# felixlutz/carla-social-force-model

Hardware: AMD Instinct MI355X
Metric: sfm_ticks_per_s (higher is better)
Workload: dtype f32

## Files before the change

carla-social-force-model_amd/csrc/sfm_capi.hip:

```cpp
#include "sfm_capi_common.h"

using namespace sfm;

constexpr int GEO_SLICES_MAX = 16;


struct DevGeo {
    DevBuf<int> off;
    DevBuf<float2> pts;
    DevBuf<float4> ctr;
    DevBuf<float4> seg;
    int K = 0;
    int P = 0;
    PinnedBuf<char> stage;
    std::vector<int> off_host;
    bool lazy = false;
    bool lazy_off = false;
};

struct FsmDev {
    bool on = false;
    int n = 0;
    DevBuf<uint8_t> mode;
    DevBuf<float> target, initial, crossing, margin, next;
// ... 830 lines not shown
    return sa;
}

constexpr int PHASE_FULL = 0, PHASE_BEGIN = 1, PHASE_END = 2;
constexpr int LIST_ALL = 0, LIST_OWN = 1, LIST_REMOTE = 2;

static int fused_launch(SfmHandle* h, uint32_t flags, int mode, int* sl) {
    const int n_g = (h->n_t + 1) / 2;
    const size_t rows = (size_t)n_g * (size_t)h->N_pad;
    TickArgs a;
    fill_args(h, a, flags);
    const bool geo = a.geo != nullptr;
    int slices = 0, nw = 16;
    const int n_pair = fused_pair_workgroups(n_g);
    if (geo) {
        slices = h->n_t <= 64 ? 4 : 2;
        if (h->n_t >= 6) slices = std::max(slices, std::min(FUSED_GEO_SLICES_MAX, (256 - n_pair) / h->n_t));
        if (n_pair + h->n_t * slices > 512) nw = 8;
    }
    const size_t grow = (size_t)FUSED_GEO_SLICES_MAX * (size_t)h->N_pad;
    if (geo && a.adv.M > 0) {
        float4* c_in = mode ? h->fused.dyn_ctr_alt : h->dynamics.ctr;
        float2* p_in = mode ? h->fused.dyn_pts_alt : h->dynamics.pts;
        a.dynamics.ctr = c_in; a.dynamics.pts = p_in;
        a.adv.ctr = c_in; a.adv.pts = p_in;
        a.adv.ctr_out = mode ? h->dynamics.ctr : h->fused.dyn_ctr_alt;
        a.adv.pts_out = mode ? h->dynamics.pts : h->fused.dyn_pts_alt;
    }
    const FusedArgs f{h->fused.fslab + (size_t)(*sl ^ 1) * rows, h->fused.fslab + (size_t)*sl * rows,
                      h->z3 ? h->fused.fslabz + (size_t)(*sl ^ 1) * rows : nullptr, h->z3 ? h->fused.fslabz + (size_t)*sl * rows : nullptr,
                      h->own, h->fused.own_alt, n_g, h->n_t, n_g % 8 == 0 ? 1 : 0,
                      geo ? h->fused.fgeo + (size_t)(*sl ^ 1) * grow : nullptr, geo ? h->fused.fgeo + (size_t)*sl * grow : nullptr, slices,
                      geo ? h->n_t * slices : 0, n_pair, mode};
    HIP_TRY(h, launch_fused_tick(h->rad, a, f, h->stream, nw));
    if (mode != 0) {
        h->cur ^= 1;
        swap(h->own, h->fused.own_alt);
        if (geo && a.adv.M > 0) {
            swap(h->dynamics.ctr, h->fused.dyn_ctr_alt);
            swap(h->dynamics.pts, h->fused.dyn_pts_alt);
        }
    }
    *sl ^= 1;
    return SFM_OK;
}

static int fused_reserve(SfmHandle* h) {
    const size_t need = (size_t)2 * (size_t)((h->n_t + 1) / 2) * (size_t)h->N_pad;
    FusedDev& f = h->fused;
    if (need > f.fslab.cap()) HIP_TRY(h, f.fslab.alloc(need));
    if (h->z3 && need > f.fslabz.cap()) HIP_TRY(h, f.fslabz.alloc(need));
    if (f.own_alt.cap() < (size_t)h->cap) HIP_TRY(h, f.own_alt.alloc((size_t)h->cap));
    const size_t gneed = (size_t)2 * FUSED_GEO_SLICES_MAX * (size_t)h->N_pad;
    if (gneed > f.fgeo.cap()) HIP_TRY(h, f.fgeo.alloc(gneed));
    if (h->dyn_boxes && h->dynamics.K > 0) {
        if (f.dyn_ctr_alt.cap() != h->dynamics.ctr.cap()) HIP_TRY(h, f.dyn_ctr_alt.alloc(h->dynamics.ctr.cap()));
        if (f.dyn_pts_alt.cap() != h->dynamics.pts.cap()) HIP_TRY(h, f.dyn_pts_alt.alloc(h->dynamics.pts.cap()));
    }
    return SFM_OK;
}

static int run_fused(SfmHandle* h, int ticks, uint32_t flags, bool carry, bool geo) {
    int rc = fused_reserve(h);
    if (rc) return rc;
    snprintf(h->variant, sizeof(h->variant), geo ? "sfm_fused_tick_kernel(geo)" : "sfm_fused_tick_kernel");
    if (h->timing_on) HIP_TRY(h, hipEventRecord(h->ev0, h->stream));
    int sl = carry ? h->carry_sl : 0;
// ... 712 lines not shown
```

carla-social-force-model_amd/csrc/sfm_capi_common.h:

```cpp
#pragma once
#include "sfm_devbuf.h"
#include "sfm_device.h"
#include "sfm_hip.h"

#include <algorithm>
#include <cmath>
#include <numeric>
#include <cstdio>
#include <cstdlib>
#include <cstring>
#include <limits>
#include <string>
#include <vector>

namespace sfm {
hipError_t launch_tick(int ipw, int team, bool z3, bool rad, const TickArgs& a, hipStream_t st);
hipError_t launch_arrived(const float4* pk, const float4* own, int N, float thr2, uint8_t* mask, hipStream_t st);
hipError_t launch_sym_list(const TickArgs& a, const SymArgs& sa, hipStream_t st, int partners = 0, bool count_is_zero = false);
hipError_t launch_sym_pair(bool rad, const TickArgs& a, const SymArgs& sa, hipStream_t st);
hipError_t launch_sym_epilogue(bool rad, const TickArgs& a, const SymArgs& sa, hipStream_t st);
hipError_t launch_fused_tick(bool rad, const TickArgs& a, const FusedArgs& f, hipStream_t st, int waves);
int fused_pair_workgroups(int n_g);
hipError_t launch_sym_pair_geo(bool rad, const TickArgs& a, const SymArgs& sa, hipStream_t st);
int sym_item_count(int n_t);
hipError_t launch_strip_bounds(const float4* box, const float* vmax, int n_t, int tps, int n_strips, float4* sbox, float* svmax,
                               hipStream_t st);
hipError_t launch_tile_strip_bounds(const float4* pk, int N, int n_t, int tps, int n_strips, float4* box, float* vmax, float4* sbox,
                                    float* svmax, hipStream_t st);
hipError_t launch_geometry(bool rad, const TickArgs& a, hipStream_t st);
hipError_t launch_modes(const TickArgs& a, hipStream_t st);
struct ReorderBufs { unsigned long long *key64_in, *key64_out; uint32_t *row_a, *row_b, *key32_in, *key32_out; void* temp; size_t temp_bytes; };
size_t reorder_temp_bytes(int N);
hipError_t launch_resort(const float4* pk, int N, int strip_rows, const ReorderBufs& b, hipStream_t st);
hipError_t launch_resort_blocks(const float4* pk, int N, const BlockPlan& pl, const ReorderBufs& b, hipStream_t st);
hipError_t launch_unpack_geo(const char* block, float4* ctr, int K, float2* pts, int P, int* off, bool with_off, hipStream_t st);
hipError_t launch_unpack_rows(const char* block, size_t b_own, size_t b_zv, size_t b_rr, size_t b_cm, int n_pad, float4* pk0,
                              float4* pk1, float4* own, float2* zv0, float2* zv1, float* radius, uint8_t* crossing, uint32_t* draws,
                              const char* geo_block, float4* ctr, int K, float2* pts, int P, int* off, bool with_off, hipStream_t st);
hipError_t launch_gather(const uint32_t* src, int N, const float4* pk_in, float4* pk_out, const float2* zv_in, float2* zv_out,
                         const float4* own_in, float4* own_out, const float* rad_in, float* rad_out, const uint8_t* cr_in,
                         uint8_t* cr_out, const uint32_t* dr_in, uint32_t* dr_out, const uint32_t* id_in, uint32_t* id_out,
                         hipStream_t st);
hipError_t launch_tile_bounds(const float4* pk, const float2* zv, int N, float4* box, float* vmax, hipStream_t st, int t_lo = 0,
                              int t_hi = -1);
int probe_dpp_direction(hipStream_t st);
hipError_t launch_batch_tick(bool z3, bool ext, bool modes, bool spawn, bool steer, const BatchArgs& a, int B, hipStream_t st);
hipError_t launch_batch_park_unborn(const int* scene_off, const uint8_t* born, float4* pk, float2* zv, int B, hipStream_t st);
hipError_t launch_batch_place_tracks(const BatchTracks& t, const int* off, const float2* local, float4* ctr, float2* pts, int M,
                                     hipStream_t st);
hipError_t launch_batch_restart(const BatchRestart& r, int scenes, hipStream_t st);
hipError_t launch_batch_observe(const ObserveArgs& a, int B, hipStream_t st);
hipError_t launch_dynamic_boxes(float4* ctr, const int* off, const float2* local, const float2* rot, float2* pts, int M,
                                float dt, int advance, hipStream_t st);

// ... 38 lines not shown
```

carla-social-force-model_amd/csrc/sfm_device.h:

```cpp
#pragma once
#include <hip/hip_runtime.h>
#include <stdint.h>

namespace sfm {

constexpr int WAVE = 64;
constexpr int BLOCK = 256;
constexpr int WAVES_PER_BLOCK = BLOCK / WAVE;
constexpr int TILE_J = BLOCK;
constexpr float TINY = 1e-30f;
constexpr float COINCIDENT_RINV = 1e14f;

constexpr float FAR_AWAY = 3.0e15f;
constexpr float FAR_STEP = 1.0e12f;
constexpr float BOX_LIMIT = 1.0e14f;
constexpr float NEAR_LIMIT = 1.0e12f;

struct IxConst {
    float lam;
    float eg;
    float c1;
    float k1;
    float k2;
    float negA;
// ... 105 lines not shown
    int t_lo, t_hi;
    int zero_count;
    uint32_t* idx;
    uint32_t row_base;
    uint32_t cap_pairs;
    struct SpillArgs* spill;
    int tick_serial;
};

struct SpillArgs {
    long long* ovf;
    int n_pad;
    int tick;
};

constexpr int FUSED_GEO_SLICES_MAX = 8;
struct alignas(16) FusedArgs {
    const float2* slab_prev;
    float2* slab_next;
    const float* slabz_prev;
    float* slabz_next;
    const float4* own_cur;
    float4* own_next;
    int n_g;
    int n_t;
    int blocked;
    const float2* geo_prev;
    float2* geo_next;
    int geo_slices;
    int n_geo_wg;
    int n_pair_wg;
    int mode;
};

constexpr int BATCH_MAX_N = 1024;
struct BatchParams {
    IxConst ped, stat, dyn;
    float border_a, border_nlb;
    float inv_tau, dt, max_speed_factor;
    int en_acc, en_ped, en_border, en_static, en_dynamic;
    int rad;
    int pad;
};
struct BatchGeo {
    const int* item_off;
    const int* off;
    const float2* pts;
    const float4* ctr;
};
struct BatchStream {
    uint32_t seed;
    float world_side;
    float arrive_thr2;
    float pad;
};
struct BatchModeScene {
    float arrive_thr2;
    float veh_ext_x, veh_ext_y;
    int despawn_on_arrival;
};
struct BatchModes {
    uint8_t* mode;
    float* target;
    const float4* speeds;
    const int* wp_off;
    const float2* wp_xy;
// ... 90 lines not shown
```

carla-social-force-model_amd/csrc/sfm_kernels.hip:

```cpp
#include "sfm_device.h"
#include "sfm_interaction.h"

#include <algorithm>
#include <type_traits>

namespace sfm {

typedef float v2f __attribute__((ext_vector_type(2)));
__device__ __forceinline__ v2f bcast(float v) { v2f r; r.x = v; r.y = v; return r; }
template <bool RAD, bool CUT>
__device__ __forceinline__ bool moussaid_planar_pk(const IxConst& c, v2f pj, v2f uj, v2f Ti, v2f Ui, float rsum, float reach2, v2f& term) {
    const v2f dd = pj - Ti;
    const float d2 = fmaf(dd.x, dd.x, dd.y * dd.y);
    if (CUT && !__any(!(d2 > reach2))) return false;
    v2f sq, rr;
    sq.x = d2;
    rr.x = rsq(d2);
    const v2f Dv = __builtin_elementwise_fma(dd, __builtin_shufflevector(rr, rr, 0, 0), Ui - uj);
    const float D2 = fmaf(Dv.x, Dv.x, fmaf(Dv.y, Dv.y, TINY));
    sq.y = D2;
    rr.y = rsq(D2);
    const float rD = rr.y;
    float aL = 0.f;
    if (CUT) {
// ... 1517 lines not shown
        rc[(3 * 3 + 0) * n + i] = fsx; rc[(3 * 3 + 1) * n + i] = fsy; rc[(3 * 3 + 2) * n + i] = 0.f;
        rc[(4 * 3 + 0) * n + i] = fdx; rc[(4 * 3 + 1) * n + i] = fdy; rc[(4 * 3 + 2) * n + i] = 0.f;
        rc[(5 * 3 + 0) * n + i] = Fx;  rc[(5 * 3 + 1) * n + i] = Fy;  rc[(5 * 3 + 2) * n + i] = Fz;
    }
}

constexpr int GROUP = 2 * WAVE;

template <bool RAD, int NW, bool Z3>
struct FusedShared {
    float4 st[2 * GROUP];
    float rad[2 * GROUP];
    float2 q[Z3 ? 1 : NW / 2][2 * GROUP];
    float2 part[2 * GROUP];
    int badrow[2 * GROUP];
    int any;
    float2 fi[NW][WAVE];
    float2 fj[NW][WAVE];
    float fiz[Z3 ? NW : 1][WAVE];
    float fjz[Z3 ? NW : 1][WAVE];
    float2 fi2[NW][WAVE];
    float fi2z[Z3 ? NW : 1][WAVE];
    float4 trav[4][2 * WAVE];
    float radt[RAD ? 4 : 1][2 * WAVE];
    float2 stz[Z3 ? 2 * GROUP : 1];
    float2 travz[Z3 ? 4 : 1][2 * WAVE];
    float partz[Z3 ? 2 * GROUP : 1];
    __device__ __forceinline__ float2 (*qv())[2 * GROUP] { return Z3 ? reinterpret_cast<float2 (*)[2 * GROUP]>(&fi[0][0]) : q; }
    __device__ __forceinline__ float (*qzv())[2 * GROUP] {
        return reinterpret_cast<float (*)[2 * GROUP]>(reinterpret_cast<char*>(&fi[0][0]) + sizeof(float2) * (NW / 2) * 2 * GROUP);
    }
};

template <bool RAD, int NW, bool Z3, bool GEO>
__global__ __launch_bounds__(NW * WAVE, (NW == 8 && Z3) ? 6 : 8) void sfm_fused_tick_kernel(const TickArgs a, const FusedArgs f) {
    constexpr int PARTS = NW / 2;
    constexpr int SPW = 4 * WAVE / NW;
    constexpr int D = NW / 8;
    using Sh = FusedShared<RAD, NW, Z3>;
    constexpr size_t LDS = (GEO && sizeof(GeoShared<NW>) > sizeof(Sh)) ? sizeof(GeoShared<NW>) : sizeof(Sh);
    __shared__ __attribute__((aligned(16))) char smem[LDS];
    Sh& sh = *reinterpret_cast<Sh*>(smem);
    static_assert(!Z3 || (offsetof(Sh, fjz) + sizeof(sh.fjz) - offsetof(Sh, fi) == (sizeof(float2) + sizeof(float)) * (NW / 2) * 2 * GROUP &&
                          offsetof(Sh, fj) == offsetof(Sh, fi) + sizeof(sh.fi) && offsetof(Sh, fiz) == offsetof(Sh, fj) + sizeof(sh.fj) &&
                          offsetof(Sh, fjz) == offsetof(Sh, fiz) + sizeof(sh.fiz)),
                  "3-D: q / qz are laid over fi | fj | fiz | fjz, which must be one block of exactly that size");
    const int tid = threadIdx.x;
    const int lane = tid & (WAVE - 1);
    const int wave = uniform(tid >> 6);
    const int n_g = f.n_g, n_t = f.n_t;
    const int half_up = (n_g + 1) >> 1;
    const bool geo_role = GEO && (int)blockIdx.x < f.n_geo_wg;
    const int bid = (int)blockIdx.x - (GEO ? f.n_geo_wg : 0);
    if (GEO && bid >= f.n_pair_wg) {
        const int k = (bid - f.n_pair_wg) * NW + wave;
        if (k < a.adv.M) advance_vehicle(a.adv, k, lane, true);
        return;
    }
    const int geo_tile = geo_role ? (int)blockIdx.x % n_t : 0, geo_slice = geo_role ? (int)blockIdx.x / n_t : 0;
    int GX, GY;
    bool diag_item;
    if (geo_role) {
        GX = geo_tile >> 1; GY = n_g;
        diag_item = false;
    } else if (f.blocked) {
        const int s = n_g >> 2;
        const int x = bid & 7;
        int k = bid >> 3;
        if (x < 6) {
            const int I = x < 3 ? 0 : (x < 5 ? 1 : 2), J = x < 3 ? x + 1 : (x < 5 ? x - 1 : 3);
            GX = I * s + k / s;
            GY = J * s + k % s;
            diag_item = false;
        } else {
            const int per_band = (s * s) >> 1;
            const int I = 2 * (x - 6) + (k >= per_band ? 1 : 0);
            if (k >= per_band) k -= per_band;
            if (k < (s >> 1)) {
                GX = I * s + 2 * k; GY = GX + 1;
                diag_item = true;
            } else {
                int t = k - (s >> 1), u = 0;
                while (t >= s - 1 - u) { t -= s - 1 - u; ++u; }
                GX = I * s + u; GY = I * s + u + 1 + t;
                diag_item = false;
            }
        }
    } else {
        int shift = 0, bx = bid;
        if (bx >= half_up) {
            const int id = bx - half_up;
            shift = 1 + id / n_g;
            bx = id - (shift - 1) * n_g;
        }
        GX = bx;
        GY = bx + (shift == 0 ? half_up : shift);
        if (shift != 0 && GY >= n_g) GY -= n_g;
        diag_item = shift == 0;
    }

    const bool integrate = f.mode != 0;
    const int quarter = wave & (2 * GROUP / WAVE - 1);
    const int p = quarter * WAVE + lane;
    const bool lower = wave < 2 * GROUP / WAVE;
    const int G = (quarter < 2) ? GX : GY;
    const bool present = G < n_g;
    const int i = G * GROUP + (quarter & 1) * WAVE + lane;
    const bool live = present && i < a.N;
    float4 st = make_float4(0.f, 0.f, 0.f, 0.f), o = st;
    float2 stz = make_float2(0.f, 0.f);
    float2 geo_f = make_float2(0.f, 0.f);
    uint32_t nd0 = 0, pid = 0;
    if (present && lower) {
        st = a.pk_cur[i];
        if (Z3) stz = a.zv_cur[i];
        if (live && integrate) {
            o = f.own_cur[i];
            if (GEO) {
                float2 gv[FUSED_GEO_SLICES_MAX];
#pragma unroll
                for (int k = 0; k < FUSED_GEO_SLICES_MAX; ++k) gv[k] = k < f.geo_slices ? f.geo_prev[(size_t)k * a.N_pad + i] : make_float2(0.f, 0.f);
                geo_f = make_float2(((gv[0].x + gv[1].x) + (gv[2].x + gv[3].x)) + ((gv[4].x + gv[5].x) + (gv[6].x + gv[7].x)),
                                    ((gv[0].y + gv[1].y) + (gv[2].y + gv[3].y)) + ((gv[4].y + gv[5].y) + (gv[6].y + gv[7].y)));
            }
            if ((a.flags & 2u) && diag_item) { nd0 = a.draws[i]; pid = a.ids ? a.ids[i] : (uint32_t)i; }
        }
        if (RAD) {
            const float r_ = a.radius[i];
            sh.rad[p] = r_;
            sh.radt[RAD ? (p >> 6) : 0][p & (WAVE - 1)] = r_; sh.radt[RAD ? (p >> 6) : 0][(p & (WAVE - 1)) + WAVE] = r_;
        }
    }
    if (tid == 0) sh.any = 0;
    {
        const int pp = (wave & 1) * WAVE + lane;
        const int part = wave >> 1;
        const int Gq = (wave & 1) ? GY : GX;
        const int i2 = Gq * GROUP + 2 * lane;
        float4 acc4 = make_float4(0.f, 0.f, 0.f, 0.f);
        float2 accz = make_float2(0.f, 0.f);
        if (integrate && a.en_ped && Gq < n_g && i2 < a.N) {
            const float4* col = reinterpret_cast<const float4*>(f.slab_prev + i2);
            const float2* colz = Z3 ? reinterpret_cast<const float2*>(f.slabz_prev + i2) : nullptr;
            const size_t stride4 = (size_t)a.N_pad / 2;
            const int per = (n_g + PARTS - 1) / PARTS;
            const int r1 = min(n_g, (part + 1) * per);
            const int r00 = part * per;
            if (!Z3 && r1 - r00 == 4) {
                const float4 v0 = col[(size_t)r00 * stride4], v1 = col[(size_t)(r00 + 1) * stride4];
                const float4 v2 = col[(size_t)(r00 + 2) * stride4], v3 = col[(size_t)(r00 + 3) * stride4];
                acc4 = make_float4((v0.x + v1.x) + (v2.x + v3.x), (v0.y + v1.y) + (v2.y + v3.y),
                                   (v0.z + v1.z) + (v2.z + v3.z), (v0.w + v1.w) + (v2.w + v3.w));
            } else if (!Z3) {
                for (int r0 = r00; r0 < r1; r0 += 8) {
                    float4 v[8];
#pragma unroll
                    for (int k = 0; k < 8; ++k) v[k] = (r0 + k < r1) ? col[(size_t)(r0 + k) * stride4] : make_float4(0.f, 0.f, 0.f, 0.f);
                    acc4.x += ((v[0].x + v[1].x) + (v[2].x + v[3].x)) + ((v[4].x + v[5].x) + (v[6].x + v[7].x));
                    acc4.y += ((v[0].y + v[1].y) + (v[2].y + v[3].y)) + ((v[4].y + v[5].y) + (v[6].y + v[7].y));
                    acc4.z += ((v[0].z + v[1].z) + (v[2].z + v[3].z)) + ((v[4].z + v[5].z) + (v[6].z + v[7].z));
                    acc4.w += ((v[0].w + v[1].w) + (v[2].w + v[3].w)) + ((v[4].w + v[5].w) + (v[6].w + v[7].w));
                }
            } else {
                for (int r0 = part * per; r0 < r1; r0 += 4) {
                    float4 v[4];
                    float2 vz[4];
#pragma unroll
                    for (int k = 0; k < 4; ++k) {
                        v[k] = (r0 + k < r1) ? col[(size_t)(r0 + k) * stride4] : make_float4(0.f, 0.f, 0.f, 0.f);
                        vz[k] = (r0 + k < r1) ? colz[(size_t)(r0 + k) * stride4] : make_float2(0.f, 0.f);
                    }
                    acc4.x += (v[0].x + v[1].x) + (v[2].x + v[3].x);
                    acc4.y += (v[0].y + v[1].y) + (v[2].y + v[3].y);
                    acc4.z += (v[0].z + v[1].z) + (v[2].z + v[3].z);
                    acc4.w += (v[0].w + v[1].w) + (v[2].w + v[3].w);
                    accz.x += (vz[0].x + vz[1].x) + (vz[2].x + vz[3].x);
                    accz.y += (vz[0].y + vz[1].y) + (vz[2].y + vz[3].y);
                }
            }
        }
        sh.qv()[part][2 * pp] = make_float2(acc4.x, acc4.y);
        sh.qv()[part][2 * pp + 1] = make_float2(acc4.z, acc4.w);
        if (Z3) { sh.qzv()[part][2 * pp] = accz.x; sh.qzv()[part][2 * pp + 1] = accz.y; }
    }
    __syncthreads();
    auto put_state = [&](const float4 ns, const float2 nsz) {
        sh.st[p] = ns;
        const float4 t = make_float4(ns.x, ns.y, a.ped.lam * ns.z, a.ped.lam * ns.w);
        float* pl = reinterpret_cast<float*>(sh.trav) + (p >> 6) * 2 * WAVE + (p & (WAVE - 1));
        pl[0] = t.x; pl[WAVE] = t.x;
        pl[8 * WAVE] = t.y; pl[9 * WAVE] = t.y;
        pl[16 * WAVE] = t.z; pl[17 * WAVE] = t.z;
        pl[24 * WAVE] = t.w; pl[25 * WAVE] = t.w;
        if (Z3) {
            sh.stz[Z3 ? p : 0] = nsz;
            const float2 tz = make_float2(nsz.x, a.ped.lam * nsz.y);
            float* plz = reinterpret_cast<float*>(sh.travz) + (p >> 6) * 2 * WAVE + (p & (WAVE - 1));
            plz[0] = tz.x; plz[WAVE] = tz.x;
            plz[8 * WAVE] = tz.y; plz[9 * WAVE] = tz.y;
        }
    };
    auto finish = [&](const float2 g, const float gz) {
        const float fpx = a.en_ped ? a.ped.negA * g.x : 0.f, fpy = a.en_ped ? a.ped.negA * g.y : 0.f;
        const float fpz = (Z3 && a.en_ped) ? a.ped.negA * gz : 0.f;
        const float x = st.x, y = st.y, vx = st.z, vy = st.w, ts = o.z;
        const float z = stz.x, vz = stz.y;
        float wx = o.x, wy = o.y;
        float fax = 0.f, fay = 0.f, faz = 0.f;
        if (a.en_acc) acceleration_force<Z3, true>(a, wx, wy, x, y, vx, vy, vz, ts, fax, fay, faz);
        const float Fx = (fax + fpx) + geo_f.x, Fy = (fay + fpy) + geo_f.y;
        const float Fz = faz + fpz;
        float nvx, nvy, nvz;
        capped_velocity<Z3, true>(a, vx, vy, vz, Fx, Fy, Fz, ts, nvx, nvy, nvz);
        float nx = x, ny = y, nz = z;
        if (a.flags & 1u) { nx = fmaf(a.dt, nvx, x); ny = fmaf(a.dt, nvy, y); if (Z3) nz = fmaf(a.dt, nvz, z); }
        const float4 ns = make_float4(nx, ny, nvx, nvy);
        const float2 nsz = make_float2(nz, nvz);
        if (diag_item) {
            if (a.flags & 2u) {
                const float ax_ = wx - x, ay_ = wy - y;
                if (fmaf(ax_, ax_, ay_ * ay_) < a.arrive_thr2) {
                    const uint32_t nd = nd0 + 1u;
                    const float2 w = next_waypoint(a.seed, pid, nd, a.world_side);
                    wx = w.x; wy = w.y;
                    a.draws[i] = nd;
                }
            }
            f.own_next[i] = make_float4(wx, wy, o.z, o.w);
            a.pk_next[i] = ns;
            if (Z3) a.zv_next[i] = nsz;
        }
        put_state(ns, nsz);
    };
    bool bad = false;
    if (lower && present) {
        if (integrate && live) {
            float2 g = sh.qv()[0][p];
            float gz = Z3 ? sh.qzv()[0][p] : 0.f;
#pragma unroll
            for (int k = 1; k < PARTS; ++k) { const float2 q = sh.qv()[k][p]; g.x += q.x; g.y += q.y; if (Z3) gz += sh.qzv()[k][p]; }
            bad = a.en_ped && (!(fabsf(g.x) < __builtin_inff()) || !(fabsf(g.y) < __builtin_inff()) || (Z3 && !(fabsf(gz) < __builtin_inff())));
            if (bad) sh.any = 1; else finish(g, gz);
        } else {
            put_state(st, stz);
        }
    }
    if (lower) sh.badrow[p] = bad ? 1 : 0;
    __syncthreads();
    if (sh.any) {
        const int N = a.N;
        for (int q = wave; q < 2 * GROUP; q += NW) {
            if (!sh.badrow[q]) continue;
            const int Gq = (q < GROUP) ? GX : GY;
            const int ip = Gq * GROUP + (q & (GROUP - 1));
            const float4 si = a.pk_cur[ip];
            const float xi = uniform(si.x), yi = uniform(si.y), vxi = uniform(si.z), vyi = uniform(si.w);
            float zi = 0.f, vzi = 0.f;
            if (Z3) { const float2 sz = a.zv_cur[ip]; zi = uniform(sz.x); vzi = uniform(sz.y); }
            float gx = 0.f, gy = 0.f, gz = 0.f;
            for (int j0 = 0; j0 < N; j0 += WAVE) {
                const int j = j0 + lane;
                const float4 pj = a.pk_cur[min(j, N - 1)];
                float2 pz = make_float2(0.f, 0.f);
                if (Z3) pz = a.zv_cur[min(j, N - 1)];
                float cx = 0.f, cy = 0.f, cz = 0.f, rinv;
                moussaid<Z3, RAD, true>(a.ped, pj.x - xi, pj.y - yi, pz.x - zi, vxi - pj.z, vyi - pj.w, vzi - pz.y,
                                        RAD ? a.radius[ip] + a.radius[min(j, N - 1)] : 0.f, cx, cy, cz, rinv);
                const bool valid = (j < N) & (j != ip);
                gx += valid ? cx : 0.f;
                gy += valid ? cy : 0.f;
                if (Z3) gz += valid ? cz : 0.f;
            }
            gx = wave_sum(gx);
            gy = wave_sum(gy);
            if (Z3) gz = wave_sum(gz);
            if (lane == 0) { sh.part[q] = make_float2(gx, gy); if (Z3) sh.partz[Z3 ? q : 0] = gz; }
        }
        __syncthreads();
        if (bad) finish(sh.part[p], Z3 ? sh.partz[Z3 ? p : 0] : 0.f);
        __syncthreads();
    }

    if (GEO && geo_role) {
        const int ig = geo_tile * WAVE + lane;
        const float4 sg = sh.st[(geo_tile & 1) * WAVE + lane];
        GeoLane me;
        me.live = ig < a.N;
        me.x = FAR_AWAY; me.y = FAR_AWAY; me.vx = 0.f; me.vy = 0.f; me.r = 0.f;
        if (me.live) { me.x = sg.x; me.y = sg.y; me.vx = sg.z; me.vy = sg.w; me.r = f.own_cur[ig].w; }
        me.walk = me.live && !(a.crossing && a.crossing[ig]);
        __syncthreads();
        GeoShared<NW>& gs = *reinterpret_cast<GeoShared<NW>*>(smem);
        geometry_forces<RAD, NW, true>(a, gs, me, geo_slice, f.geo_slices, tid);
        if (wave < 2 && me.live) {
            float vb = 0.f, vs = 0.f, vd = 0.f;
#pragma unroll
            for (int w = 0; w < NW; ++w) { vb += gs.acc[w][wave][lane]; vs += gs.acc[w][2 + wave][lane]; vd += gs.acc[w][4 + wave][lane]; }
            reinterpret_cast<float*>(f.geo_next + (size_t)geo_slice * a.N_pad + ig)[wave] = (vb + a.stat.negA * vs) + a.dyn.negA * vd;
        }
        return;
    }

    int ia, ib, sig0;
    bool diag = false, work = true;
    if (diag_item) {
        const int sel = wave / (NW / 2);
        const int lw = wave % (NW / 2);
        const int base = sel * GROUP;
        const int Gd = sel ? GY : GX;
        if (lw < 2 * D) {
            const int tl = lw / D;
            ia = ib = base + tl * WAVE;
            sig0 = 1 + (lw % D) * SPW;
            diag = true;
            work = Gd < n_g && 2 * Gd + tl < n_t;
        } else {
            ia = base; ib = base + WAVE;
            sig0 = (lw - 2 * D) * SPW;
            work = Gd < n_g && 2 * Gd + 1 < n_t;
        }
    } else {
        const int q = wave / (NW / 4);
        ia = (q >> 1) * WAVE;
        ib = GROUP + (q & 1) * WAVE;
        sig0 = (wave % (NW / 4)) * SPW;
        work = 2 * GX + (q >> 1) < n_t && 2 * GY + (q & 1) < n_t;
    }
    float fxi = 0.f, fyi = 0.f, fxj = 0.f, fyj = 0.f, fzi = 0.f, fzj = 0.f;
    int i_end_loc = lane;
    float fxb = 0.f, fyb = 0.f, fzb = 0.f;
    int i_end_b = lane;
    if (work) {
        const IxConst& c = a.ped;
        const float4 pj = sh.st[ib + lane];
        const float ujx = c.lam * pj.z, ujy = c.lam * pj.w;
        float zj = 0.f, ujz = 0.f;
        if (Z3) { const float2 qz = sh.stz[Z3 ? ib + lane : 0]; zj = qz.x; ujz = c.lam * qz.y; }
        float rj = 0.f;
        if (RAD) rj = sh.rad[ib + lane];
        constexpr int HALF = SPW / 2;
        const int s0 = diag ? 1 + ((sig0 - 1) >> 1) : sig0 >> 1;
        const float* pl = reinterpret_cast<const float*>(sh.trav) + (ia >> 6) * 2 * WAVE + lane + s0;
        const float* plz = reinterpret_cast<const float*>(sh.travz) + (Z3 ? (ia >> 6) * 2 * WAVE + lane + s0 : 0);
        const float* plr = &sh.radt[RAD ? (ia >> 6) : 0][RAD ? lane + s0 : 0];
        v2f fjx = bcast(0.f), fjy = bcast(0.f), fjzv = bcast(0.f);
        auto chain = [&](auto xb_tag) __attribute__((always_inline)) {
            constexpr int XB = decltype(xb_tag)::value;
            const bool tail_one_sided = diag && (s0 + XB + HALF - 1 == 32);
            v2f X, Y, U, V;
            X.x = pl[0]; X.y = pl[XB]; Y.x = pl[8 * WAVE]; Y.y = pl[8 * WAVE + XB];
            U.x = pl[16 * WAVE]; U.y = pl[16 * WAVE + XB]; V.x = pl[24 * WAVE]; V.y = pl[24 * WAVE + XB];
            v2f Zp = bcast(0.f), Wp = bcast(0.f), Rp = bcast(0.f);
            if (Z3) { Zp.x = plz[0]; Zp.y = plz[XB]; Wp.x = plz[8 * WAVE]; Wp.y = plz[8 * WAVE + XB]; }
            if (RAD) { Rp.x = plr[0]; Rp.y = plr[XB]; }
#pragma unroll
            for (int s_ = 0; s_ < HALF; ++s_) {
                constexpr bool PRE = !(Z3 && NW == 16);
                if (!PRE && s_ > 0) {
                    X.x = pl[s_]; X.y = pl[s_ + XB]; Y.x = pl[8 * WAVE + s_]; Y.y = pl[8 * WAVE + s_ + XB];
                    U.x = pl[16 * WAVE + s_]; U.y = pl[16 * WAVE + s_ + XB]; V.x = pl[24 * WAVE + s_]; V.y = pl[24 * WAVE + s_ + XB];
                    if (Z3) { Zp.x = plz[s_]; Zp.y = plz[s_ + XB]; Wp.x = plz[8 * WAVE + s_]; Wp.y = plz[8 * WAVE + s_ + XB]; }
                    if (RAD) { Rp.x = plr[s_]; Rp.y = plr[s_ + XB]; }
                }
                v2f Xn = X, Yn = Y, Un = U, Vn = V, Zn = Zp, Wn = Wp, Rn = Rp;
                if (PRE && s_ + 1 < HALF) {
                    Xn.x = pl[s_ + 1]; Xn.y = pl[s_ + 1 + XB]; Yn.x = pl[8 * WAVE + s_ + 1]; Yn.y = pl[8 * WAVE + s_ + 1 + XB];
                    Un.x = pl[16 * WAVE + s_ + 1]; Un.y = pl[16 * WAVE + s_ + 1 + XB]; Vn.x = pl[24 * WAVE + s_ + 1]; Vn.y = pl[24 * WAVE + s_ + 1 + XB];
                    if (Z3) { Zn.x = plz[s_ + 1]; Zn.y = plz[s_ + 1 + XB]; Wn.x = plz[8 * WAVE + s_ + 1]; Wn.y = plz[8 * WAVE + s_ + 1 + XB]; }
                    if (RAD) { Rn.x = plr[s_ + 1]; Rn.y = plr[s_ + 1 + XB]; }
                }
                __builtin_amdgcn_sched_barrier(0);
                v2f cx, cy, cz = bcast(0.f);
                if (Z3) moussaid_spatial_x2<RAD>(c, pj.x, pj.y, zj, ujx, ujy, ujz, X, Y, Zp, U, V, Wp, cx, cy, cz, Rp + bcast(rj));
                else moussaid_planar_x2<RAD>(c, pj.x, pj.y, ujx, ujy, X, Y, U, V, cx, cy, Rp + bcast(rj));
                fxi = rot_in(fxi) + cx.x; fyi = rot_in(fyi) + cy.x;
                fxb = rot_in(fxb) + cx.y; fyb = rot_in(fyb) + cy.y;
                if (Z3) { fzi = rot_in(fzi) + cz.x; fzb = rot_in(fzb) + cz.y; }
                if (s_ + 1 == HALF && tail_one_sided) { fjx.x -= cx.x; fjy.x -= cy.x; if (Z3) fjzv.x -= cz.x; }
                else { fjx -= cx; fjy -= cy; if (Z3) fjzv -= cz; }
                X = Xn; Y = Yn; U = Un; V = Vn; Zp = Zn; Wp = Wn; Rp = Rn;
                __builtin_amdgcn_sched_barrier(0);
            }
            i_end_loc = (lane + s0 + HALF - 1) & (WAVE - 1);
            i_end_b = (lane + s0 + XB + HALF - 1) & (WAVE - 1);
        };
        if (diag) chain(std::integral_constant<int, 16>{});
        else chain(std::integral_constant<int, 32>{});
        fxj = fjx.x + fjx.y;
        fyj = fjy.x + fjy.y;
        if (Z3) fzj = fjzv.x + fjzv.y;
    }
    sh.fi[wave][i_end_loc] = make_float2(fxi, fyi);
    sh.fi2[wave][i_end_b] = make_float2(fxb, fyb);
    if (Z3) sh.fi2z[Z3 ? wave : 0][i_end_b] = fzb;
    sh.fj[wave][lane] = make_float2(fxj, fyj);
    if (Z3) { sh.fiz[Z3 ? wave : 0][i_end_loc] = fzi; sh.fjz[Z3 ? wave : 0][lane] = fzj; }
    __syncthreads();
    if (!lower || !present) return;
    const int tl = (p >> 6) & 1, l = lane;
    auto fi = [&](int w) {
        float2 v = sh.fi[w][l];
        const float2 v2 = sh.fi2[w][l]; v.x += v2.x; v.y += v2.y;
        float vz_ = Z3 ? sh.fiz[Z3 ? w : 0][l] : 0.f;
        if (Z3) vz_ += sh.fi2z[Z3 ? w : 0][l];
        return make_float3(v.x, v.y, vz_);
    };
    auto fj = [&](int w) { const float2 v = sh.fj[w][l]; return make_float3(v.x, v.y, Z3 ? sh.fjz[Z3 ? w : 0][l] : 0.f); };
    float3 r = make_float3(0.f, 0.f, 0.f);
    int row;
    if (diag_item) {
        const int w0 = (p < GROUP) ? 0 : NW / 2;
#pragma unroll
        for (int k = 0; k < D; ++k) {
            const float3 u = fi(w0 + tl * D + k), v = fj(w0 + tl * D + k);
            r.x += u.x + v.x; r.y += u.y + v.y; r.z += u.z + v.z;
        }
#pragma unroll
        for (int k = 0; k < 2 * D; ++k) {
            const float3 u = tl ? fj(w0 + 2 * D + k) : fi(w0 + 2 * D + k);
            r.x += u.x; r.y += u.y; r.z += u.z;
        }
        row = G;
    } else if (p < GROUP) {
#pragma unroll
        for (int k = 0; k < NW / 2; ++k) { const float3 u = fi(tl * (NW / 2) + k); r.x += u.x; r.y += u.y; r.z += u.z; }
        row = GY;
    } else {
#pragma unroll
        for (int h = 0; h < 2; ++h)
#pragma unroll
            for (int k = 0; k < NW / 4; ++k) { const float3 u = fj((2 * h + tl) * (NW / 4) + k); r.x += u.x; r.y += u.y; r.z += u.z; }
        row = GX;
    }
    f.slab_next[(size_t)row * a.N_pad + i] = make_float2(r.x, r.y);
    if (Z3) f.slabz_next[(size_t)row * a.N_pad + i] = r.z;
}

__global__ __launch_bounds__(BLOCK) void sfm_dynamic_boxes_kernel(float4* __restrict__ ctr, const int* __restrict__ off,
                                                                  const float2* __restrict__ local, const float2* __restrict__ rot,
                                                                  float2* __restrict__ pts, int M, float dt, int advance) {
    const int k = blockIdx.x * WAVES_PER_BLOCK + (int)(threadIdx.x >> 6);
    if (k >= M) return;
    advance_vehicle(DynAdvance{ctr, off, local, rot, pts, M, dt, 0, nullptr, nullptr}, k, threadIdx.x & (WAVE - 1), advance != 0);
}

__global__ void sfm_arrived_kernel(const float4* __restrict__ pk, const float4* __restrict__ own, int N, float thr2,
                                   uint8_t* __restrict__ mask) {
    const int i = blockIdx.x * blockDim.x + threadIdx.x;
    if (i >= N) return;
    const float4 s = pk[i];
    const float4 o = own[i];
    const float ddx = o.x - s.x, ddy = o.y - s.y;
    mask[i] = fmaf(ddx, ddx, ddy * ddy) < thr2 ? 1 : 0;
}

template <int IPW, bool Z3, bool RAD, int TEAM>
static hipError_t launch_one(const TickArgs& a, hipStream_t st) {
    const int n_local = a.i_end - a.i_begin;
    if (n_local <= 0) return hipSuccess;
    const int per_block = IPW * (WAVES_PER_BLOCK / TEAM);
    const int grid = (n_local + per_block - 1) / per_block;
    TickArgs b = a;
    b.adv.block0 = grid;
    const int extra = a.adv.M > 0 ? (a.adv.M + WAVES_PER_BLOCK - 1) / WAVES_PER_BLOCK : 0;
    hipLaunchKernelGGL((sfm_tick_kernel<IPW, Z3, RAD, TEAM>), dim3(grid + extra), dim3(BLOCK), 0, st, b);
    return hipGetLastError();
}

// ... 115 lines not shown
    hipLaunchKernelGGL(sfm_tile_strip_bounds_kernel, dim3(n_strips), dim3(TSB_WAVES * WAVE), 0, st, pk, N, n_t, tps, box, vmax, sbox, svmax);
    return hipGetLastError();
}

hipError_t launch_strip_bounds(const float4* box, const float* vmax, int n_t, int tps, int n_strips, float4* sbox, float* svmax,
                               hipStream_t st) {
    if (n_strips <= 0) return hipSuccess;
    hipLaunchKernelGGL(sfm_strip_bounds_kernel, dim3(n_strips), dim3(WAVE), 0, st, box, vmax, n_t, tps, sbox, svmax);
    return hipGetLastError();
}

template <bool RAD, int EW>
static void launch_sym_epilogue_t(const TickArgs& a, const SymArgs& sa, hipStream_t st) {
    TickArgs b = a;
    SymArgs sb = sa;
    b.adv.block0 = sa.t_hi - sa.t_lo;
    const int extra = a.adv.M > 0 ? (a.adv.M + EW - 1) / EW : 0;
    const dim3 grid(sa.t_hi - sa.t_lo + extra);
    if (sa.slabz) hipLaunchKernelGGL((sfm_sym_epilogue_kernel<RAD, EW, true>), grid, dim3(EW * WAVE), 0, st, b, sb);
    else hipLaunchKernelGGL((sfm_sym_epilogue_kernel<RAD, EW, false>), grid, dim3(EW * WAVE), 0, st, b, sb);
}

hipError_t launch_sym_epilogue(bool rad, const TickArgs& a, const SymArgs& sa, hipStream_t st) {
    if (a.N <= 0) return hipSuccess;
    const bool thin = sa.n_t >= 1024;
    if (rad) { if (thin) launch_sym_epilogue_t<true, 4>(a, sa, st); else launch_sym_epilogue_t<true, EPI_WAVES>(a, sa, st); }
    else { if (thin) launch_sym_epilogue_t<false, 4>(a, sa, st); else launch_sym_epilogue_t<false, EPI_WAVES>(a, sa, st); }
    return hipGetLastError();
}

int fused_pair_workgroups(int n_g) { return (n_g + 1) / 2 + n_g * ((n_g - 1) / 2) + ((n_g & 1) ? 0 : n_g / 2); }

template <bool RAD, int NW>
static void launch_fused_t(dim3 grid, bool geo, bool z3, const TickArgs& a, const FusedArgs& f, hipStream_t st) {
    if (z3) {
        if (geo) hipLaunchKernelGGL((sfm_fused_tick_kernel<RAD, NW, true, true>), grid, dim3(NW * WAVE), 0, st, a, f);
        else hipLaunchKernelGGL((sfm_fused_tick_kernel<RAD, NW, true, false>), grid, dim3(NW * WAVE), 0, st, a, f);
    } else {
        if (geo) hipLaunchKernelGGL((sfm_fused_tick_kernel<RAD, NW, false, true>), grid, dim3(NW * WAVE), 0, st, a, f);
        else hipLaunchKernelGGL((sfm_fused_tick_kernel<RAD, NW, false, false>), grid, dim3(NW * WAVE), 0, st, a, f);
    }
}

hipError_t launch_fused_tick(bool rad, const TickArgs& a, const FusedArgs& f, hipStream_t st, int nw) {
    if (a.N <= 1 || f.n_g < 1) return hipErrorInvalidValue;
    const bool geo = f.n_geo_wg > 0, z3 = f.slabz_next != nullptr;
    const int n_adv = (geo && a.adv.M > 0) ? (a.adv.M + nw - 1) / nw : 0;
    const dim3 grid(f.n_geo_wg + f.n_pair_wg + n_adv);
    if (nw == 8) { if (rad) launch_fused_t<true, 8>(grid, geo, z3, a, f, st); else launch_fused_t<false, 8>(grid, geo, z3, a, f, st); }
    else { if (rad) launch_fused_t<true, 16>(grid, geo, z3, a, f, st); else launch_fused_t<false, 16>(grid, geo, z3, a, f, st); }
    return hipGetLastError();
}

int probe_dpp_direction(hipStream_t st) {
    int* d = nullptr;
    if (hipMalloc(reinterpret_cast<void**>(&d), 64 * sizeof(int)) != hipSuccess) return 0;
    hipLaunchKernelGGL(sfm_dpp_probe_kernel, dim3(1), dim3(64), 0, st, d);
    int h[64];
    hipError_t e = hipMemcpy(h, d, sizeof(h), hipMemcpyDeviceToHost);
    hipFree(d);
    if (e != hipSuccess) return 0;
    bool up = true, down = true;
    for (int l = 0; l < 64; ++l) { up &= (h[l] == ((l + 1) & 63)); down &= (h[l] == ((l + 63) & 63)); }
    return up ? 1 : (down ? -1 : 0);
}

hipError_t launch_dynamic_boxes(float4* ctr, const int* off, const float2* local, const float2* rot, float2* pts, int M,
                                float dt, int advance, hipStream_t st) {
    if (M <= 0) return hipSuccess;
    hipLaunchKernelGGL(sfm_dynamic_boxes_kernel, dim3((M + WAVES_PER_BLOCK - 1) / WAVES_PER_BLOCK), dim3(BLOCK), 0, st, ctr, off, local,
                       rot, pts, M, dt, advance);
    return hipGetLastError();
}

hipError_t launch_arrived(const float4* pk, const float4* own, int N, float thr2, uint8_t* mask, hipStream_t st) {
    if (N <= 0) return hipSuccess;
    hipLaunchKernelGGL(sfm_arrived_kernel, dim3((N + 255) / 256), dim3(256), 0, st, pk, own, N, thr2, mask);
    return hipGetLastError();
}

}
```

Measured before the change: 64850.

## Pack hot kernel arguments up front and stage wave priority through pair loop

Adds a 64-byte-aligned FusedHot struct holding the frequently used pointers and scalars and passes it as the first kernel argument. Empty asm statements force those values into scalar registers so fewer kernarg loads sit on the critical path. The fused kernel also raises wave priority with s_setprio at entry, steps it down in stages across the pair-interaction loop, and raises it again for the reduction. The aim is to cut argument-load latency and to let waves nearing completion of the compute loop yield to waves in their load or reduction phases. In exchange, more SGPRs are pinned, which could add register pressure, and the priority staging may disturb the scheduling balance.

Result: no change. 65490, median of 6 (+1.0%).

```diff
diff --git a/carla-social-force-model_amd/csrc/sfm_capi.hip b/carla-social-force-model_amd/csrc/sfm_capi.hip
--- a/carla-social-force-model_amd/csrc/sfm_capi.hip
+++ b/carla-social-force-model_amd/csrc/sfm_capi.hip
@@ -886,7 +886,10 @@
                       h->own, h->fused.own_alt, n_g, h->n_t, n_g % 8 == 0 ? 1 : 0,
                       geo ? h->fused.fgeo + (size_t)(*sl ^ 1) * grow : nullptr, geo ? h->fused.fgeo + (size_t)*sl * grow : nullptr, slices,
                       geo ? h->n_t * slices : 0, n_pair, mode};
-    HIP_TRY(h, launch_fused_tick(h->rad, a, f, h->stream, nw));
+    const FusedHot hot{a.pk_cur, a.pk_next, f.own_cur, f.own_next, f.slab_prev, f.slab_next, a.draws, a.ids, a.radius,
+                       a.N, a.N_pad, a.flags, a.en_acc, a.en_ped, f.n_g, f.n_t, f.blocked, f.mode, f.n_geo_wg, f.n_pair_wg,
+                       a.inv_tau, a.dt, a.max_speed_factor, a.seed, a.world_side, a.arrive_thr2, a.ped};
+    HIP_TRY(h, launch_fused_tick(h->rad, hot, a, f, h->stream, nw));
     if (mode != 0) {
         h->cur ^= 1;
         swap(h->own, h->fused.own_alt);
diff --git a/carla-social-force-model_amd/csrc/sfm_capi_common.h b/carla-social-force-model_amd/csrc/sfm_capi_common.h
--- a/carla-social-force-model_amd/csrc/sfm_capi_common.h
+++ b/carla-social-force-model_amd/csrc/sfm_capi_common.h
@@ -19,7 +19,7 @@
 hipError_t launch_sym_list(const TickArgs& a, const SymArgs& sa, hipStream_t st, int partners = 0, bool count_is_zero = false);
 hipError_t launch_sym_pair(bool rad, const TickArgs& a, const SymArgs& sa, hipStream_t st);
 hipError_t launch_sym_epilogue(bool rad, const TickArgs& a, const SymArgs& sa, hipStream_t st);
-hipError_t launch_fused_tick(bool rad, const TickArgs& a, const FusedArgs& f, hipStream_t st, int waves);
+hipError_t launch_fused_tick(bool rad, const FusedHot& h, const TickArgs& a, const FusedArgs& f, hipStream_t st, int waves);
 int fused_pair_workgroups(int n_g);
 hipError_t launch_sym_pair_geo(bool rad, const TickArgs& a, const SymArgs& sa, hipStream_t st);
 int sym_item_count(int n_t);
diff --git a/carla-social-force-model_amd/csrc/sfm_device.h b/carla-social-force-model_amd/csrc/sfm_device.h
--- a/carla-social-force-model_amd/csrc/sfm_device.h
+++ b/carla-social-force-model_amd/csrc/sfm_device.h
@@ -161,6 +161,26 @@
     int n_pair_wg;
     int mode;
 };
+struct alignas(64) FusedHot {
+    const float4* pk_cur;
+    float4* pk_next;
+    const float4* own_cur;
+    float4* own_next;
+    const float2* slab_prev;
+    float2* slab_next;
+    uint32_t* draws;
+    const uint32_t* ids;
+    const float* radius;
+    int N, N_pad;
+    uint32_t flags;
+    int en_acc, en_ped;
+    int n_g, n_t, blocked, mode, n_geo_wg, n_pair_wg;
+    float inv_tau, dt, max_speed_factor;
+    uint32_t seed;
+    float world_side, arrive_thr2;
+    IxConst ped;
+};
+static_assert(alignof(FusedHot) == 64 && sizeof(FusedHot) <= 192, "FusedHot: three 64-byte lines at the front of the kernel arguments");
 
 constexpr int BATCH_MAX_N = 1024;
 struct BatchParams {
diff --git a/carla-social-force-model_amd/csrc/sfm_kernels.hip b/carla-social-force-model_amd/csrc/sfm_kernels.hip
--- a/carla-social-force-model_amd/csrc/sfm_kernels.hip
+++ b/carla-social-force-model_amd/csrc/sfm_kernels.hip
@@ -1573,8 +1573,22 @@
     }
 };
 
+__device__ constexpr int step_level(int s, int half) {
+    const int k = s * 8 / half;
+    return k < 3 ? 3 : k < 5 ? 2 : k < 7 ? 1 : 0;
+}
+template <int HALF>
+__device__ __forceinline__ void step_priority(int s) {
+    const int lv = step_level(s, HALF);
+    if (s != 0 && lv == step_level(s - 1, HALF)) return;
+    if (lv == 3) __builtin_amdgcn_s_setprio(3);
+    else if (lv == 2) __builtin_amdgcn_s_setprio(2);
+    else if (lv == 1) __builtin_amdgcn_s_setprio(1);
+    else __builtin_amdgcn_s_setprio(0);
+}
+
 template <bool RAD, int NW, bool Z3, bool GEO>
-__global__ __launch_bounds__(NW * WAVE, (NW == 8 && Z3) ? 6 : 8) void sfm_fused_tick_kernel(const TickArgs a, const FusedArgs f) {
+__global__ __launch_bounds__(NW * WAVE, (NW == 8 && Z3) ? 6 : 8) void sfm_fused_tick_kernel(const FusedHot hot, const TickArgs a, const FusedArgs f) {
     constexpr int PARTS = NW / 2;
     constexpr int SPW = 4 * WAVE / NW;
     constexpr int D = NW / 8;
@@ -1586,15 +1600,24 @@
                           offsetof(Sh, fj) == offsetof(Sh, fi) + sizeof(sh.fi) && offsetof(Sh, fiz) == offsetof(Sh, fj) + sizeof(sh.fj) &&
                           offsetof(Sh, fjz) == offsetof(Sh, fiz) + sizeof(sh.fiz)),
                   "3-D: q / qz are laid over fi | fj | fiz | fjz, which must be one block of exactly that size");
+    constexpr bool PRIO = !(GEO && NW == 16);
+    if (PRIO) __builtin_amdgcn_s_setprio(3);
+    const FusedHot& h = hot;
+    asm volatile("" :: "s"(h.pk_cur), "s"(h.pk_next), "s"(h.own_cur), "s"(h.own_next), "s"(h.slab_prev), "s"(h.slab_next),
+                       "s"(h.draws), "s"(h.ids), "s"(h.radius), "s"(h.N), "s"(h.N_pad), "s"(h.flags), "s"(h.en_acc), "s"(h.en_ped),
+                       "s"(h.n_g), "s"(h.n_t), "s"(h.blocked), "s"(h.mode), "s"(h.n_geo_wg), "s"(h.n_pair_wg),
+                       "s"(h.inv_tau), "s"(h.dt), "s"(h.max_speed_factor), "s"(h.seed), "s"(h.world_side), "s"(h.arrive_thr2),
+                       "s"(h.ped.lam), "s"(h.ped.eg), "s"(h.ped.c1), "s"(h.ped.k1));
+    asm volatile("" :: "s"(h.ped.k2), "s"(h.ped.negA));
     const int tid = threadIdx.x;
     const int lane = tid & (WAVE - 1);
     const int wave = uniform(tid >> 6);
-    const int n_g = f.n_g, n_t = f.n_t;
+    const int n_g = h.n_g, n_t = h.n_t;
     const int half_up = (n_g + 1) >> 1;
-    const bool geo_role = GEO && (int)blockIdx.x < f.n_geo_wg;
-    const int bid = (int)blockIdx.x - (GEO ? f.n_geo_wg : 0);
-    if (GEO && bid >= f.n_pair_wg) {
-        const int k = (bid - f.n_pair_wg) * NW + wave;
+    const bool geo_role = GEO && (int)blockIdx.x < h.n_geo_wg;
+    const int bid = (int)blockIdx.x - (GEO ? h.n_geo_wg : 0);
+    if (GEO && bid >= h.n_pair_wg) {
+        const int k = (bid - h.n_pair_wg) * NW + wave;
         if (k < a.adv.M) advance_vehicle(a.adv, k, lane, true);
         return;
     }
@@ -1604,7 +1627,7 @@
     if (geo_role) {
         GX = geo_tile >> 1; GY = n_g;
         diag_item = false;
-    } else if (f.blocked) {
+    } else if (h.blocked) {
         const int s = n_g >> 2;
         const int x = bid & 7;
         int k = bid >> 3;
@@ -1640,34 +1663,34 @@
         diag_item = shift == 0;
     }
 
-    const bool integrate = f.mode != 0;
+    const bool integrate = h.mode != 0;
     const int quarter = wave & (2 * GROUP / WAVE - 1);
     const int p = quarter * WAVE + lane;
     const bool lower = wave < 2 * GROUP / WAVE;
     const int G = (quarter < 2) ? GX : GY;
     const bool present = G < n_g;
     const int i = G * GROUP + (quarter & 1) * WAVE + lane;
-    const bool live = present && i < a.N;
+    const bool live = present && i < h.N;
     float4 st = make_float4(0.f, 0.f, 0.f, 0.f), o = st;
     float2 stz = make_float2(0.f, 0.f);
     float2 geo_f = make_float2(0.f, 0.f);
     uint32_t nd0 = 0, pid = 0;
     if (present && lower) {
-        st = a.pk_cur[i];
+        st = h.pk_cur[i];
         if (Z3) stz = a.zv_cur[i];
         if (live && integrate) {
-            o = f.own_cur[i];
+            o = h.own_cur[i];
             if (GEO) {
                 float2 gv[FUSED_GEO_SLICES_MAX];
 #pragma unroll
-                for (int k = 0; k < FUSED_GEO_SLICES_MAX; ++k) gv[k] = k < f.geo_slices ? f.geo_prev[(size_t)k * a.N_pad + i] : make_float2(0.f, 0.f);
+                for (int k = 0; k < FUSED_GEO_SLICES_MAX; ++k) gv[k] = k < f.geo_slices ? f.geo_prev[(size_t)k * h.N_pad + i] : make_float2(0.f, 0.f);
                 geo_f = make_float2(((gv[0].x + gv[1].x) + (gv[2].x + gv[3].x)) + ((gv[4].x + gv[5].x) + (gv[6].x + gv[7].x)),
                                     ((gv[0].y + gv[1].y) + (gv[2].y + gv[3].y)) + ((gv[4].y + gv[5].y) + (gv[6].y + gv[7].y)));
             }
-            if ((a.flags & 2u) && diag_item) { nd0 = a.draws[i]; pid = a.ids ? a.ids[i] : (uint32_t)i; }
+            if ((h.flags & 2u) && diag_item) { nd0 = h.draws[i]; pid = h.ids ? h.ids[i] : (uint32_t)i; }
         }
         if (RAD) {
-            const float r_ = a.radius[i];
+            const float r_ = h.radius[i];
             sh.rad[p] = r_;
             sh.radt[RAD ? (p >> 6) : 0][p & (WAVE - 1)] = r_; sh.radt[RAD ? (p >> 6) : 0][(p & (WAVE - 1)) + WAVE] = r_;
         }
@@ -1680,10 +1703,10 @@
         const int i2 = Gq * GROUP + 2 * lane;
         float4 acc4 = make_float4(0.f, 0.f, 0.f, 0.f);
         float2 accz = make_float2(0.f, 0.f);
-        if (integrate && a.en_ped && Gq < n_g && i2 < a.N) {
-            const float4* col = reinterpret_cast<const float4*>(f.slab_prev + i2);
+        if (integrate && h.en_ped && Gq < n_g && i2 < h.N) {
+            const float4* col = reinterpret_cast<const float4*>(h.slab_prev + i2);
             const float2* colz = Z3 ? reinterpret_cast<const float2*>(f.slabz_prev + i2) : nullptr;
-            const size_t stride4 = (size_t)a.N_pad / 2;
+            const size_t stride4 = (size_t)h.N_pad / 2;
             const int per = (n_g + PARTS - 1) / PARTS;
             const int r1 = min(n_g, (part + 1) * per);
             const int r00 = part * per;
@@ -1727,7 +1750,7 @@
     __syncthreads();
     auto put_state = [&](const float4 ns, const float2 nsz) {
         sh.st[p] = ns;
-        const float4 t = make_float4(ns.x, ns.y, a.ped.lam * ns.z, a.ped.lam * ns.w);
+        const float4 t = make_float4(ns.x, ns.y, h.ped.lam * ns.z, h.ped.lam * ns.w);
         float* pl = reinterpret_cast<float*>(sh.trav) + (p >> 6) * 2 * WAVE + (p & (WAVE - 1));
         pl[0] = t.x; pl[WAVE] = t.x;
         pl[8 * WAVE] = t.y; pl[9 * WAVE] = t.y;
@@ -1735,40 +1758,40 @@
         pl[24 * WAVE] = t.w; pl[25 * WAVE] = t.w;
         if (Z3) {
             sh.stz[Z3 ? p : 0] = nsz;
-            const float2 tz = make_float2(nsz.x, a.ped.lam * nsz.y);
+            const float2 tz = make_float2(nsz.x, h.ped.lam * nsz.y);
             float* plz = reinterpret_cast<float*>(sh.travz) + (p >> 6) * 2 * WAVE + (p & (WAVE - 1));
             plz[0] = tz.x; plz[WAVE] = tz.x;
             plz[8 * WAVE] = tz.y; plz[9 * WAVE] = tz.y;
         }
     };
     auto finish = [&](const float2 g, const float gz) {
-        const float fpx = a.en_ped ? a.ped.negA * g.x : 0.f, fpy = a.en_ped ? a.ped.negA * g.y : 0.f;
-        const float fpz = (Z3 && a.en_ped) ? a.ped.negA * gz : 0.f;
+        const float fpx = h.en_ped ? h.ped.negA * g.x : 0.f, fpy = h.en_ped ? h.ped.negA * g.y : 0.f;
+        const float fpz = (Z3 && h.en_ped) ? h.ped.negA * gz : 0.f;
         const float x = st.x, y = st.y, vx = st.z, vy = st.w, ts = o.z;
         const float z = stz.x, vz = stz.y;
         float wx = o.x, wy = o.y;
         float fax = 0.f, fay = 0.f, faz = 0.f;
-        if (a.en_acc) acceleration_force<Z3, true>(a, wx, wy, x, y, vx, vy, vz, ts, fax, fay, faz);
+        if (h.en_acc) acceleration_force<Z3, true>(h, wx, wy, x, y, vx, vy, vz, ts, fax, fay, faz);
         const float Fx = (fax + fpx) + geo_f.x, Fy = (fay + fpy) + geo_f.y;
         const float Fz = faz + fpz;
         float nvx, nvy, nvz;
-        capped_velocity<Z3, true>(a, vx, vy, vz, Fx, Fy, Fz, ts, nvx, nvy, nvz);
+        capped_velocity<Z3, true>(h, vx, vy, vz, Fx, Fy, Fz, ts, nvx, nvy, nvz);
         float nx = x, ny = y, nz = z;
-        if (a.flags & 1u) { nx = fmaf(a.dt, nvx, x); ny = fmaf(a.dt, nvy, y); if (Z3) nz = fmaf(a.dt, nvz, z); }
+        if (h.flags & 1u) { nx = fmaf(h.dt, nvx, x); ny = fmaf(h.dt, nvy, y); if (Z3) nz = fmaf(h.dt, nvz, z); }
         const float4 ns = make_float4(nx, ny, nvx, nvy);
         const float2 nsz = make_float2(nz, nvz);
         if (diag_item) {
-            if (a.flags & 2u) {
+            if (h.flags & 2u) {
                 const float ax_ = wx - x, ay_ = wy - y;
-                if (fmaf(ax_, ax_, ay_ * ay_) < a.arrive_thr2) {
+                if (fmaf(ax_, ax_, ay_ * ay_) < h.arrive_thr2) {
                     const uint32_t nd = nd0 + 1u;
-                    const float2 w = next_waypoint(a.seed, pid, nd, a.world_side);
+                    const float2 w = next_waypoint(h.seed, pid, nd, h.world_side);
                     wx = w.x; wy = w.y;
-                    a.draws[i] = nd;
+                    h.draws[i] = nd;
                 }
             }
-            f.own_next[i] = make_float4(wx, wy, o.z, o.w);
-            a.pk_next[i] = ns;
+            h.own_next[i] = make_float4(wx, wy, o.z, o.w);
+            h.pk_next[i] = ns;
             if (Z3) a.zv_next[i] = nsz;
         }
         put_state(ns, nsz);
@@ -1780,7 +1803,7 @@
             float gz = Z3 ? sh.qzv()[0][p] : 0.f;
 #pragma unroll
             for (int k = 1; k < PARTS; ++k) { const float2 q = sh.qv()[k][p]; g.x += q.x; g.y += q.y; if (Z3) gz += sh.qzv()[k][p]; }
-            bad = a.en_ped && (!(fabsf(g.x) < __builtin_inff()) || !(fabsf(g.y) < __builtin_inff()) || (Z3 && !(fabsf(gz) < __builtin_inff())));
+            bad = h.en_ped && (!(fabsf(g.x) < __builtin_inff()) || !(fabsf(g.y) < __builtin_inff()) || (Z3 && !(fabsf(gz) < __builtin_inff())));
             if (bad) sh.any = 1; else finish(g, gz);
         } else {
             put_state(st, stz);
@@ -1789,24 +1812,24 @@
     if (lower) sh.badrow[p] = bad ? 1 : 0;
     __syncthreads();
     if (sh.any) {
-        const int N = a.N;
+        const int N = h.N;
         for (int q = wave; q < 2 * GROUP; q += NW) {
             if (!sh.badrow[q]) continue;
             const int Gq = (q < GROUP) ? GX : GY;
             const int ip = Gq * GROUP + (q & (GROUP - 1));
-            const float4 si = a.pk_cur[ip];
+            const float4 si = h.pk_cur[ip];
             const float xi = uniform(si.x), yi = uniform(si.y), vxi = uniform(si.z), vyi = uniform(si.w);
             float zi = 0.f, vzi = 0.f;
             if (Z3) { const float2 sz = a.zv_cur[ip]; zi = uniform(sz.x); vzi = uniform(sz.y); }
             float gx = 0.f, gy = 0.f, gz = 0.f;
             for (int j0 = 0; j0 < N; j0 += WAVE) {
                 const int j = j0 + lane;
-                const float4 pj = a.pk_cur[min(j, N - 1)];
+                const float4 pj = h.pk_cur[min(j, N - 1)];
                 float2 pz = make_float2(0.f, 0.f);
                 if (Z3) pz = a.zv_cur[min(j, N - 1)];
                 float cx = 0.f, cy = 0.f, cz = 0.f, rinv;
-                moussaid<Z3, RAD, true>(a.ped, pj.x - xi, pj.y - yi, pz.x - zi, vxi - pj.z, vyi - pj.w, vzi - pz.y,
-                                        RAD ? a.radius[ip] + a.radius[min(j, N - 1)] : 0.f, cx, cy, cz, rinv);
+                moussaid<Z3, RAD, true>(h.ped, pj.x - xi, pj.y - yi, pz.x - zi, vxi - pj.z, vyi - pj.w, vzi - pz.y,
+                                        RAD ? h.radius[ip] + h.radius[min(j, N - 1)] : 0.f, cx, cy, cz, rinv);
                 const bool valid = (j < N) & (j != ip);
                 gx += valid ? cx : 0.f;
                 gy += valid ? cy : 0.f;
@@ -1826,9 +1849,9 @@
         const int ig = geo_tile * WAVE + lane;
         const float4 sg = sh.st[(geo_tile & 1) * WAVE + lane];
         GeoLane me;
-        me.live = ig < a.N;
+        me.live = ig < h.N;
         me.x = FAR_AWAY; me.y = FAR_AWAY; me.vx = 0.f; me.vy = 0.f; me.r = 0.f;
-        if (me.live) { me.x = sg.x; me.y = sg.y; me.vx = sg.z; me.vy = sg.w; me.r = f.own_cur[ig].w; }
+        if (me.live) { me.x = sg.x; me.y = sg.y; me.vx = sg.z; me.vy = sg.w; me.r = h.own_cur[ig].w; }
         me.walk = me.live && !(a.crossing && a.crossing[ig]);
         __syncthreads();
         GeoShared<NW>& gs = *reinterpret_cast<GeoShared<NW>*>(smem);
@@ -1837,7 +1860,7 @@
             float vb = 0.f, vs = 0.f, vd = 0.f;
 #pragma unroll
             for (int w = 0; w < NW; ++w) { vb += gs.acc[w][wave][lane]; vs += gs.acc[w][2 + wave][lane]; vd += gs.acc[w][4 + wave][lane]; }
-            reinterpret_cast<float*>(f.geo_next + (size_t)geo_slice * a.N_pad + ig)[wave] = (vb + a.stat.negA * vs) + a.dyn.negA * vd;
+            reinterpret_cast<float*>(f.geo_next + (size_t)geo_slice * h.N_pad + ig)[wave] = (vb + a.stat.negA * vs) + a.dyn.negA * vd;
         }
         return;
     }
@@ -1872,7 +1895,7 @@
     float fxb = 0.f, fyb = 0.f, fzb = 0.f;
     int i_end_b = lane;
     if (work) {
-        const IxConst& c = a.ped;
+        const IxConst& c = h.ped;
         const float4 pj = sh.st[ib + lane];
         const float ujx = c.lam * pj.z, ujy = c.lam * pj.w;
         float zj = 0.f, ujz = 0.f;
@@ -1911,6 +1934,7 @@
                     if (RAD) { Rn.x = plr[s_ + 1]; Rn.y = plr[s_ + 1 + XB]; }
                 }
                 __builtin_amdgcn_sched_barrier(0);
+                if (PRIO) step_priority<HALF>(s_);
                 v2f cx, cy, cz = bcast(0.f);
                 if (Z3) moussaid_spatial_x2<RAD>(c, pj.x, pj.y, zj, ujx, ujy, ujz, X, Y, Zp, U, V, Wp, cx, cy, cz, Rp + bcast(rj));
                 else moussaid_planar_x2<RAD>(c, pj.x, pj.y, ujx, ujy, X, Y, U, V, cx, cy, Rp + bcast(rj));
@@ -1937,6 +1961,7 @@
     sh.fj[wave][lane] = make_float2(fxj, fyj);
     if (Z3) { sh.fiz[Z3 ? wave : 0][i_end_loc] = fzi; sh.fjz[Z3 ? wave : 0][lane] = fzj; }
     __syncthreads();
+    if (PRIO) __builtin_amdgcn_s_setprio(3);
     if (!lower || !present) return;
     const int tl = (p >> 6) & 1, l = lane;
     auto fi = [&](int w) {
@@ -1973,8 +1998,8 @@
             for (int k = 0; k < NW / 4; ++k) { const float3 u = fj((2 * h + tl) * (NW / 4) + k); r.x += u.x; r.y += u.y; r.z += u.z; }
         row = GX;
     }
-    f.slab_next[(size_t)row * a.N_pad + i] = make_float2(r.x, r.y);
-    if (Z3) f.slabz_next[(size_t)row * a.N_pad + i] = r.z;
+    h.slab_next[(size_t)row * h.N_pad + i] = make_float2(r.x, r.y);
+    if (Z3) f.slabz_next[(size_t)row * h.N_pad + i] = r.z;
 }
 
 __global__ __launch_bounds__(BLOCK) void sfm_dynamic_boxes_kernel(float4* __restrict__ ctr, const int* __restrict__ off,
@@ -2156,23 +2181,23 @@
 int fused_pair_workgroups(int n_g) { return (n_g + 1) / 2 + n_g * ((n_g - 1) / 2) + ((n_g & 1) ? 0 : n_g / 2); }
 
 template <bool RAD, int NW>
-static void launch_fused_t(dim3 grid, bool geo, bool z3, const TickArgs& a, const FusedArgs& f, hipStream_t st) {
+static void launch_fused_t(dim3 grid, bool geo, bool z3, const FusedHot& h, const TickArgs& a, const FusedArgs& f, hipStream_t st) {
     if (z3) {
-        if (geo) hipLaunchKernelGGL((sfm_fused_tick_kernel<RAD, NW, true, true>), grid, dim3(NW * WAVE), 0, st, a, f);
-        else hipLaunchKernelGGL((sfm_fused_tick_kernel<RAD, NW, true, false>), grid, dim3(NW * WAVE), 0, st, a, f);
+        if (geo) hipLaunchKernelGGL((sfm_fused_tick_kernel<RAD, NW, true, true>), grid, dim3(NW * WAVE), 0, st, h, a, f);
+        else hipLaunchKernelGGL((sfm_fused_tick_kernel<RAD, NW, true, false>), grid, dim3(NW * WAVE), 0, st, h, a, f);
     } else {
-        if (geo) hipLaunchKernelGGL((sfm_fused_tick_kernel<RAD, NW, false, true>), grid, dim3(NW * WAVE), 0, st, a, f);
-        else hipLaunchKernelGGL((sfm_fused_tick_kernel<RAD, NW, false, false>), grid, dim3(NW * WAVE), 0, st, a, f);
-    }
-}
-
-hipError_t launch_fused_tick(bool rad, const TickArgs& a, const FusedArgs& f, hipStream_t st, int nw) {
+        if (geo) hipLaunchKernelGGL((sfm_fused_tick_kernel<RAD, NW, false, true>), grid, dim3(NW * WAVE), 0, st, h, a, f);
+        else hipLaunchKernelGGL((sfm_fused_tick_kernel<RAD, NW, false, false>), grid, dim3(NW * WAVE), 0, st, h, a, f);
+    }
+}
+
+hipError_t launch_fused_tick(bool rad, const FusedHot& h, const TickArgs& a, const FusedArgs& f, hipStream_t st, int nw) {
     if (a.N <= 1 || f.n_g < 1) return hipErrorInvalidValue;
     const bool geo = f.n_geo_wg > 0, z3 = f.slabz_next != nullptr;
     const int n_adv = (geo && a.adv.M > 0) ? (a.adv.M + nw - 1) / nw : 0;
     const dim3 grid(f.n_geo_wg + f.n_pair_wg + n_adv);
-    if (nw == 8) { if (rad) launch_fused_t<true, 8>(grid, geo, z3, a, f, st); else launch_fused_t<false, 8>(grid, geo, z3, a, f, st); }
-    else { if (rad) launch_fused_t<true, 16>(grid, geo, z3, a, f, st); else launch_fused_t<false, 16>(grid, geo, z3, a, f, st); }
+    if (nw == 8) { if (rad) launch_fused_t<true, 8>(grid, geo, z3, h, a, f, st); else launch_fused_t<false, 8>(grid, geo, z3, h, a, f, st); }
+    else { if (rad) launch_fused_t<true, 16>(grid, geo, z3, h, a, f, st); else launch_fused_t<false, 16>(grid, geo, z3, h, a, f, st); }
     return hipGetLastError();
 }
 
```
